# smoggy-P/gym-Drone2D-ActivePerception

Measured on AMD Instinct MI355X. Metric: env-steps/sec (batched) at 10 agents, map_id=1, higher is better.
Workload: dtype f64

## Files before the change

gym-drone2d-activeperception_amd/csrc/d2d_hip.hip:

```cpp
#include <hip/hip_runtime.h>
#include <math.h>
#include <stdint.h>
#include <stdio.h>
#include <stdlib.h>
#include <string.h>
#include <type_traits>

#if defined(__HIP_DEVICE_COMPILE__)
#define D2D_AS __attribute__((address_space(1)))
#endif
#include "../../include/d2d.h"
#include "../../include/d2d_hooks.h"
#include "../../include/d2d_stepped.h"
#include "../../include/d2d_swept.h"

#define D2D_TAN_QUAL __device__ __forceinline__
#define D2D_TAN_TBL_QUAL __device__ const
#include "d2d_tan.h"
#define D2D_LOG_QUAL __device__ __forceinline__
#define D2D_LOG_TBL_QUAL __device__ const
#define D2D_RNG_QUAL __device__ __forceinline__
#include "d2d_rng.h"

#define WAVE 64
// ... 1885 lines not shown
  }
}

__global__ __launch_bounds__(WAVE *WAVES_PER_BLOCK) void k_reset(d2d_cfg c, d2d_state s, d2d_state init,
                                                                 const unsigned char *mask, int mask_stride) {
  const int lane = threadIdx.x & (WAVE - 1), wv = threadIdx.x / WAVE;
  const int e = blockIdx.x * WAVES_PER_BLOCK + wv;
  if (e >= c.B) return;
  if (mask && !mask[(size_t)e * mask_stride]) return;
  reset_env(c, s, init, (size_t)e, lane);
}

__global__ void k_tan(const double *in, double *out, long long n) {
  const long long i = (long long)blockIdx.x * blockDim.x + threadIdx.x;
  if (i < n) out[i] = d2d_tan(in[i]);
}

__global__ void k_log(const double *x, double *out, long long n) {
  const long long i = (long long)blockIdx.x * blockDim.x + threadIdx.x;
  if (i < n) out[i] = d2d_log(x[i]);
}

__global__ __launch_bounds__(WAVE) void k_rng_draw(uint32_t *rng, const int *m, double *out, int max_m) {
  const int lane = threadIdx.x;
  uint32_t *st = rng + (size_t)blockIdx.x * D2D_RNG_WORDS;
  double *o = out + (size_t)blockIdx.x * max_m * 2;
  const int mb = __builtin_amdgcn_readfirstlane(min(max(m[blockIdx.x], 0), max_m));
  int pos = __builtin_amdgcn_readfirstlane((int)st[D2D_RNG_POS]);
  const bool bad = !rng_pos_ok(pos);
  int got = 0, regen = 0;
  if (!bad)
    got = rng_wave_pairs(st, pos, regen, d2d_rng_regen_cap(mb), mb, lane, [&](int q, double v0, double v1) {
      o[(size_t)q * 2] = v0;
      o[(size_t)q * 2 + 1] = v1;
    });
  for (int k = got + lane; k < max_m; k += WAVE) o[(size_t)k * 2] = o[(size_t)k * 2 + 1] = k < mb ? __builtin_nan("") : 0.0;
  if (!bad) rng_wave_store(st, pos, got, regen, lane);
}

#include "d2d_plugins.h"

__global__ void k_atan2(const double *y, const double *x, double *out, long long n) {
  const long long i = (long long)blockIdx.x * blockDim.x + threadIdx.x;
  if (i < n) out[i] = d2d_atan2(y[i], x[i]);
}

struct ClosedArgs {
  d2d_cfg c;
  d2d_state s;
  d2d_plan p;
  d2d_state init;
  int on_done, nsteps;
  int obs_every;
};
static_assert(sizeof(ClosedArgs) <= D2D_LAUNCH_ARGS_BYTES, "d2d_plan.launch_args (D2D_LAUNCH_ARGS_BYTES) is too small for the parked launch arguments");

__global__ void k_closed_args(ClosedArgs *dst, d2d_cfg c, d2d_state s, d2d_plan p, d2d_state init, int on_done, int nsteps, int obs_every) {
  if (threadIdx.x == 0 && blockIdx.x == 0) {
    dst->c = c;
    dst->s = s;
    dst->p = p;
    dst->init = init;
    dst->on_done = on_done;
    dst->nsteps = nsteps;
    dst->obs_every = obs_every;
  }
}

template <int SPEC>
__host__ __device__ inline int closed_wave_bytes(const d2d_cfg &c, const d2d_plan &p, int wpb) {
  int b = make_geom(c, wpb, spec_ncap(SPEC), spec_full(SPEC)).wave_bytes;
  const int pb = plan_wave_bytes(c.N, p.nu, p.n_sample, c.W, c.H), gb = p.gaze == D2D_GAZE_OXFORD ? gaze_geom(c, p).wave_bytes : 0;
  b = b > pb ? b : pb;
  b = b > gb ? b : gb;
  return (b + 15) & ~15;
}


#if defined(__HIP_DEVICE_COMPILE__)
typedef const ClosedArgs __attribute__((address_space(4))) *ArgsPtr;
#else
typedef const ClosedArgs *ArgsPtr;
#endif

struct PhaseIn {
  ArgsPtr a;
  int e, off, lane;
};
__device__ __forceinline__ PhaseIn phase_enter(const ClosedArgs *ap, int e_, int lds_off_) {
  const unsigned long long v = (unsigned long long)ap;
  unsigned int lo = __builtin_amdgcn_readfirstlane((unsigned int)v), hi = __builtin_amdgcn_readfirstlane((unsigned int)(v >> 32));
  int e = __builtin_amdgcn_readfirstlane(e_), off = __builtin_amdgcn_readfirstlane(lds_off_);
  int lane = threadIdx.x & (WAVE - 1);
  asm volatile("; phase" : "+s"(lo), "+s"(hi), "+s"(e), "+s"(off), "+v"(lane));
  PhaseIn in;
  in.a = (ArgsPtr)(((unsigned long long)hi << 32) | lo);
  in.e = e;
  in.off = off;
  in.lane = lane;
  return in;
}
template <bool PDEF, typename F>
__device__ __forceinline__ auto with_plan(ArgsPtr a, F f) {
  if constexpr (PDEF) {
    d2d_plan p = a->p;
    plan_default_apply(p);
    return f(p);
  } else {
    return f(a->p);
  }
}


template <int SPEC, bool PDEF>
__device__ __forceinline__ int ph_plan_quick(const ClosedArgs *ap, int e_, int lds_off_) {
  const PhaseIn in_ = phase_enter(ap, e_, lds_off_);
  const ArgsPtr a = in_.a;
  const int e = in_.e, lane = in_.lane;
  char *base = d2d_lds + in_.off;
  d2d_cfg c = a->c;
  if (!spec_generic(SPEC)) spec_default_apply(c);
  if constexpr (SPEC == 1 || SPEC == 2) {
    constexpr int cap = spec_ncap(SPEC);
    __builtin_assume(c.N <= cap);
  }
  const bool need = with_plan<PDEF>(a, [&](const d2d_plan &p) __attribute__((always_inline)) { return plan_env_quick(c, a->s, p, e, lane, base); });
  wave_sync_global();
  return need ? 1 : 0;
}

template <int SPEC, bool PDEF>
__device__ __forceinline__ void ph_plan_search(const ClosedArgs *ap, int e_, int lds_off_) {
  const PhaseIn in_ = phase_enter(ap, e_, lds_off_);
  const ArgsPtr a = in_.a;
  const int e = in_.e, lane = in_.lane;
  char *base = d2d_lds + in_.off;
  d2d_cfg c = a->c;
  if (!spec_generic(SPEC)) spec_default_apply(c);
  if constexpr (SPEC == 1 || SPEC == 2) {
    constexpr int cap = spec_ncap(SPEC);
    __builtin_assume(c.N <= cap);
  }
  with_plan<PDEF>(a, [&](const d2d_plan &p) __attribute__((always_inline)) { plan_env_search<PDEF>(c, a->s, p, e, lane, base); });
  wave_sync_global();
}

__host__ __device__ constexpr uint32_t hidden_stages(uint32_t stages) { return stages & ~(uint32_t)D2D_ST_OBS; }
__host__ __device__ constexpr bool late_obs_of(uint32_t stages) { return (stages & D2D_ST_COLLIDE) && !(stages & D2D_ST_OBS); }


template <int SPEC, bool PDEF, uint32_t ACT = D2D_ST_ACT>
__device__ __forceinline__ int ph_plan_act(const ClosedArgs *ap, int e_, int lds_off_, int &walls_ok) {
  const PhaseIn in_ = phase_enter(ap, e_, lds_off_);
  const ArgsPtr a = in_.a;
  const int e = in_.e, lane = in_.lane;
  char *base = d2d_lds + in_.off;
  d2d_cfg c = a->c;
  if (!spec_generic(SPEC)) spec_default_apply(c);
  if constexpr (SPEC == 1 || SPEC == 2) {
    constexpr int cap = spec_ncap(SPEC);
    __builtin_assume(c.N <= cap);
  }
  double4 w_head;
  int wk = __builtin_amdgcn_readfirstlane(walls_ok);
  asm volatile("; phase" : "+s"(wk));
  const bool need = with_plan<PDEF>(a, [&](const d2d_plan &p) __attribute__((always_inline)) { return plan_env_quick(c, a->s, p, e, lane, base, &w_head, &wk); });
  walls_ok = __builtin_amdgcn_readfirstlane(wk);
  if (need) {
    wave_sync_global();
    return -1;
  }
  wave_sync_lds();
  StepIn in;
  in.action = 0.0;
  in.ok = true;
  in.has_wp = true;
  in.wp[0] = w_head.x; in.wp[1] = w_head.y; in.wp[2] = w_head.z; in.wp[3] = w_head.w; in.wp[4] = 0.0; in.wp[5] = 0.0;
  const int wpb = (int)(blockDim.x / WAVE);
  const Geom g = make_geom(c, wpb, spec_ncap(SPEC), spec_full(SPEC));
  const LdsView L = carve(base, g, c.L);
  EnvRegs r;
  run_env<spec_full(SPEC), spec_wide(SPEC), spec_cone(SPEC), spec_tiled(SPEC)>(c, a->s, e, lane, ACT, g, L, a->s.action[e], r, 0, true, &in, late_obs_of(ACT));
  if (lane == 0) store_regs(a->s, e, r);
  wave_sync_global();
  return r.done;
}

template <int SPEC, bool PDEF, uint32_t STAGES>
__device__ __forceinline__ int ph_gaze_stages(const ClosedArgs *ap, int e_, int lds_off_, int t_, int done_, int &dyn_gate, bool dyn_vis_) {
  const PhaseIn in_ = phase_enter(ap, e_, lds_off_);
  const ArgsPtr a = in_.a;
  const int e = in_.e, lane = in_.lane;
  int tstep = __builtin_amdgcn_readfirstlane(t_), known_done = __builtin_amdgcn_readfirstlane(done_);
  asm volatile("; phase" : "+s"(tstep), "+s"(known_done));
  int dgate = 2;
  const int dvis = dyn_vis_ ? 1 : 0;
  if constexpr (spec_full(SPEC)) {
    dgate = __builtin_amdgcn_readfirstlane(dyn_gate);
    asm volatile("; phase" : "+s"(dgate));
  }
  char *base = d2d_lds + in_.off;
  d2d_cfg c = a->c;
  if (!spec_generic(SPEC)) spec_default_apply(c);
#ifdef D2D_CHAIN_PROF
  const unsigned long long pp0 = __builtin_amdgcn_s_memtime();
#endif
  with_plan<PDEF>(a, [&](const d2d_plan &p) __attribute__((always_inline)) {
    gaze_env<true, PDEF>(c, a->s, p, a->init, a->on_done == D2D_DONE_RESET, e, lane, base, known_done);
  });
  wave_sync_global();
#ifdef D2D_CHAIN_PROF
  D2D_PHASE_ADD(0, pp0);
  const unsigned long long pp1 = __builtin_amdgcn_s_memtime();
#endif
  const int wpb = (int)(blockDim.x / WAVE);
  const Geom g = make_geom(c, wpb, spec_ncap(SPEC), spec_full(SPEC));
  const LdsView L = carve(base, g, c.L);
  EnvRegs r;
  load_regs(a->s, e, r);
  const size_t noise_off = c.noise_rows > 1 ? (size_t)((c.noise_row0 + tstep) % c.noise_rows) * c.B * c.N * 2 : 0;
  if constexpr (spec_full(SPEC)) {
    run_env<true, spec_wide(SPEC), spec_cone(SPEC), spec_tiled(SPEC)>(c, a->s, e, lane, STAGES, g, L, a->s.action[e], r, noise_off, false, nullptr, late_obs_of(STAGES), &dgate, dvis != 0, dgate == 1 && dvis == 0);
    dyn_gate = __builtin_amdgcn_readfirstlane(dgate);
  } else {
    run_env<spec_full(SPEC), spec_wide(SPEC), spec_cone(SPEC), spec_tiled(SPEC)>(c, a->s, e, lane, STAGES, g, L, a->s.action[e], r, noise_off, false, nullptr, late_obs_of(STAGES));
  }
  if (lane == 0) store_regs(a->s, e, r);
  wave_sync_global();
#ifdef D2D_CHAIN_PROF
  D2D_PHASE_ADD(1, pp1);
#endif
  return r.done;
}

template <int SPEC, uint32_t STAGES>
__device__ __forceinline__ int ph_stages(const ClosedArgs *ap, int e_, int lds_off_) {
  const PhaseIn in_ = phase_enter(ap, e_, lds_off_);
  const ArgsPtr a = in_.a;
  const int e = in_.e, lane = in_.lane;
  char *base = d2d_lds + in_.off;
  d2d_cfg c = a->c;
  if (!spec_generic(SPEC)) spec_default_apply(c);
  const int wpb = (int)(blockDim.x / WAVE);
  const Geom g = make_geom(c, wpb, spec_ncap(SPEC), spec_full(SPEC));
  const LdsView L = carve(base, g, c.L);
  EnvRegs r;
  run_env<spec_full(SPEC), spec_wide(SPEC), spec_cone(SPEC), spec_tiled(SPEC)>(c, a->s, e, lane, STAGES, g, L, a->s.action[e], r, 0, true, nullptr, late_obs_of(STAGES));
  if (lane == 0) store_regs(a->s, e, r);
  wave_sync_global();
  return r.done;
}

template <int SPEC, bool PDEF = false>
__global__ __launch_bounds__(WAVE *WAVES_PER_BLOCK, D2D_MIN_WAVES) void k_closed(const ClosedArgs *__restrict__ a) {
  static_assert(!PDEF || SPEC == 1, "the plan's defaults are folded into the few-agent kernel of the default geometry only");
  const int wv = __builtin_amdgcn_readfirstlane(threadIdx.x / WAVE);
  const int wpb = (int)(blockDim.x / WAVE);
  const int e = blockIdx.x * wpb + wv;
  if (e >= a->c.B) return;
  d2d_cfg c = a->c;
  if (!spec_generic(SPEC)) spec_default_apply(c);
  int off;
  bool split;
  if constexpr (PDEF) {
    d2d_plan p = a->p;
    plan_default_apply(p);
    off = wv * closed_wave_bytes<SPEC>(c, p, wpb);
    split = p.planner == D2D_PLAN_PRIMITIVE;
  } else {
    off = wv * closed_wave_bytes<SPEC>(c, a->p, wpb);
    split = a->p.planner == D2D_PLAN_PRIMITIVE;
  }
  const int nsteps = a->nsteps;
  const bool freeze = a->on_done == D2D_DONE_FREEZE;
  const bool obs_every = a->obs_every != 0;
  const bool dyn_defer = spec_full(SPEC) && !obs_every && !freeze, auto_reset = a->on_done == D2D_DONE_RESET;
  int dyn_gate = dyn_defer ? 0 : 2;
  int nsearch = 0;
  int walls_ok = 0;
#ifdef D2D_CHAIN_PROF
  const unsigned long long cp0 = __builtin_amdgcn_s_memtime();
  unsigned long long cps = 0;
#endif
  int flag_done = a->s.flags[(size_t)e * 4 + D2D_F_DONE] != 0 ? 1 : 0;
#pragma unroll 1
  for (int t = 0; t < nsteps; ++t) {
    if (freeze && flag_done != 0) break;
    const bool visible = obs_every || t == nsteps - 1;
    if (dyn_defer && auto_reset && flag_done != 0) dyn_gate = 0;
    if (split) {
      if (nsearch * 32 > t + 16) __builtin_amdgcn_s_setprio(2); else __builtin_amdgcn_s_setprio(0);
      ph_gaze_stages<SPEC, PDEF, D2D_ST_PERCEIVE>(a, e, off, t, flag_done, dyn_gate, visible);
#ifdef D2D_CHAIN_PROF
      const unsigned long long q0 = __builtin_amdgcn_s_memtime();
#endif
      const int pa = __builtin_amdgcn_readfirstlane(visible ? ph_plan_act<SPEC, PDEF, D2D_ST_ACT>(a, e, off, walls_ok)
                                                            : ph_plan_act<SPEC, PDEF, hidden_stages(D2D_ST_ACT)>(a, e, off, walls_ok));
#ifdef D2D_CHAIN_PROF
      D2D_PHASE_ADD(2, q0);
#endif
      if (pa < 0) {
#ifdef D2D_CHAIN_PROF
        const unsigned long long s0 = __builtin_amdgcn_s_memtime();
#endif
        ph_plan_search<SPEC, PDEF>(a, e, off);
        nsearch += 1;
        walls_ok = 0;
#ifdef D2D_CHAIN_PROF
        cps += __builtin_amdgcn_s_memtime() - s0;
        D2D_PHASE_ADD(3, s0);
        const unsigned long long a0 = __builtin_amdgcn_s_memtime();
#endif
        flag_done = __builtin_amdgcn_readfirstlane(visible ? ph_stages<SPEC, D2D_ST_ACT>(a, e, off)
                                                           : ph_stages<SPEC, hidden_stages(D2D_ST_ACT)>(a, e, off));
#ifdef D2D_CHAIN_PROF
        D2D_PHASE_ADD(4, a0);
#endif
      } else {
        flag_done = pa;
      }
    } else {
      flag_done = __builtin_amdgcn_readfirstlane(visible ? ph_gaze_stages<SPEC, PDEF, D2D_ST_ALL>(a, e, off, t, flag_done, dyn_gate, true)
                                                         : ph_gaze_stages<SPEC, PDEF, hidden_stages(D2D_ST_ALL)>(a, e, off, t, flag_done, dyn_gate, false));
    }
  }
#ifdef D2D_CHAIN_PROF
  if ((threadIdx.x & (WAVE - 1)) == 0 && a->p.plan_stat) {
    const unsigned long long tot = __builtin_amdgcn_s_memtime() - cp0;
    a->p.plan_stat[(size_t)e * 4 + 1] = (int)(tot >> 4);
    a->p.plan_stat[(size_t)e * 4 + 2] = (int)(cps >> 4);
  }
#endif
}

#include "d2d_swept.h"

thread_local char g_err[256] = "";

int fail(int code, const char *msg) {
  snprintf(g_err, sizeof g_err, "%s", msg);
  return code;
}

constexpr size_t LDS_SOFT = 64 * 1024, LDS_HARD = 160 * 1024;

template <typename K>
void lds_optin(K kernel, size_t bytes) {
  if (bytes > LDS_SOFT) (void)hipFuncSetAttribute((const void *)kernel, hipFuncAttributeMaxDynamicSharedMemorySize, (int)bytes);
}

int launched() {
  const hipError_t err = hipGetLastError();
  return err == hipSuccess ? 0 : fail(-3, hipGetErrorString(err));
}

dim3 env_grid(int B, int wpb = WAVES_PER_BLOCK) { return dim3((B + wpb - 1) / wpb); }
dim3 env_block(int wpb = WAVES_PER_BLOCK) { return dim3(WAVE * wpb); }

// ... 286 lines not shown

int d2d_reset(const d2d_cfg *c, const d2d_state *s, const d2d_state *init, const uint8_t *mask, void *stream) {
  return reset_launch(c, s, init, mask, 1, stream);
}

int d2d_gaze_stage(const d2d_cfg *c, const d2d_state *s, const d2d_plan *p, void *stream) {
  int rc = plan_check(c, s, p);
  if (rc) return rc;
  return gaze_launch(c, s, p, nullptr, false, stream);
}

int d2d_plan_stage(const d2d_cfg *c, const d2d_state *s, const d2d_plan *p, void *stream) {
  int rc = plan_check(c, s, p);
  if (rc) return rc;
  return plan_launch(c, s, p, false, stream);
}

int d2d_gaze_stage_live(const d2d_cfg *c, const d2d_state *s, const d2d_plan *p, void *stream) {
  int rc = plan_check(c, s, p);
  if (rc) return rc;
  return gaze_launch(c, s, p, nullptr, true, stream);
}

int d2d_plan_stage_live(const d2d_cfg *c, const d2d_state *s, const d2d_plan *p, void *stream) {
  int rc = plan_check(c, s, p);
  if (rc) return rc;
  return plan_launch(c, s, p, true, stream);
}

#define D2D_SWEPT_ENTRY_POINTS
#include "d2d_swept.h"

int d2d_plan_reset(const d2d_cfg *c, const d2d_plan *p, const uint8_t *mask, int32_t mask_stride, void *stream) {
  if (!c || !p) return fail(-1, "null cfg/plan");
  if (c->abi_version != D2D_ABI_VERSION) return fail(-2, "ABI version mismatch");
  return plan_reset_launch(c, p, mask, mask_stride, stream);
}

int d2d_closed_loop(const d2d_cfg *c, const d2d_state *s, const d2d_plan *p, int32_t nsteps, int32_t on_done,
                    const d2d_state *init, void *stream) {
  int rc = plan_check(c, s, p);
  if (rc) return rc;
  if (nsteps < 0) return fail(-1, "closed_loop: bad step count");
  if (on_done < D2D_DONE_CONTINUE || on_done > D2D_DONE_FREEZE) return fail(-1, "closed_loop: bad on_done");
  const bool auto_reset = on_done == D2D_DONE_RESET;
  if (auto_reset && !snapshot_complete(init)) return fail(-1, "closed_loop: D2D_DONE_RESET needs the snapshot");
  if (c->B == 0 || nsteps == 0) return 0;
  if (c->planner_mode == D2D_PLANNER_EXTERNAL && p->launch_args && (p->planner == D2D_PLAN_PRIMITIVE || p->gaze != D2D_GAZE_NONE)) {
    const Launch l = pick_launch(*c, p);
    if (l.wpb >= 1) {
      ClosedArgs *dev = (ClosedArgs *)p->launch_args;
      const char *obs_env = getenv("D2D_OBS_EVERY_STEP");
      const bool obs_every = obs_env && obs_env[0] == '1' && obs_env[1] == '\0';
      hipLaunchKernelGGL(k_closed_args, dim3(1), dim3(64), 0, (hipStream_t)stream, dev, *c, *s, *p, auto_reset ? *init : *s,
                         (int)on_done, (int)nsteps, obs_every ? 1 : 0);
      auto launch = [&](auto kernel) {
        lds_optin(kernel, l.lds());
        hipLaunchKernelGGL(kernel, env_grid(c->B, l.wpb), env_block(l.wpb), l.lds(), (hipStream_t)stream, (const ClosedArgs *)dev);
      };
      const char *fold_env = getenv("D2D_PLAN_FOLD");
      const bool fold_off = fold_env && fold_env[0] == '0' && fold_env[1] == '\0';
      if (l.spec == 1 && !fold_off && plan_default_matches(*c, *p)) launch(k_closed<1, true>);
      else with_spec(l.spec, [&](auto S) { launch(k_closed<decltype(S)::value>); });
      return launched();
    }
  }
  const bool split = p->planner == D2D_PLAN_PRIMITIVE;
  const uint32_t skip = on_done == D2D_DONE_FREEZE ? D2D_ST_SKIP_DONE : 0;
  for (int32_t t = 0; t < nsteps; ++t) {
    if ((rc = gaze_launch(c, s, p, auto_reset ? init : nullptr, skip != 0, stream))) return rc;
    d2d_state sn = *s;
    sn.noise = noise_row(c, s, t);
    if (split) {
      if ((rc = launch_stages(c, &sn, D2D_ST_PERCEIVE | skip, stream))) return rc;
      if ((rc = plan_launch(c, s, p, skip != 0, stream))) return rc;
      if ((rc = launch_stages(c, s, D2D_ST_ACT | skip, stream))) return rc;
    } else if ((rc = launch_stages(c, &sn, D2D_ST_ALL | skip, stream))) {
      return rc;
    }
  }
  return 0;
}

int d2d_launch_shape(const d2d_cfg *c, const d2d_plan *p, int32_t out[4]) {
  if (!c || !out) return fail(-1, "launch_shape: null argument");
  if (c->abi_version != D2D_ABI_VERSION) return fail(-2, "ABI version mismatch");
  Launch l = pick_launch(*c, p);
  if (p && (!p->launch_args || c->planner_mode != D2D_PLANNER_EXTERNAL)) l.wpb = 0;
  out[0] = l.wpb;
  out[1] = (int32_t)l.lds();
  out[2] = out[1] > 0 ? (int32_t)(LDS_HARD / (size_t)out[1]) : 0;
  out[3] = spec_full(l.spec) ? 1 : 0;
  return 0;
}

int d2d_sincos_array(const double *in, double *so, double *co, int64_t n, void *stream) {
  return launch_array(k_sincos, n, n > 0 && (!in || !so || !co), "sincos_array: bad arguments", stream, in, so, co);
}

int d2d_tan_array(const double *in, double *out, int64_t n, void *stream) {
  return launch_array(k_tan, n, n > 0 && (!in || !out), "tan_array: bad arguments", stream, in, out);
}

int d2d_atan2_array(const double *y, const double *x, double *out, int64_t n, void *stream) {
  return launch_array(k_atan2, n, n > 0 && (!y || !x || !out), "atan2_array: bad arguments", stream, y, x, out);
}

int d2d_log_array(const double *x, double *out, int64_t n, void *stream) {
// ... 16 lines not shown
```

gym-drone2d-activeperception_amd/csrc/d2d_plugins.h:

```cpp

#define D2D_SINCOS_QUAL __device__ __forceinline__
#define D2D_SINCOS_TBL_QUAL __device__ const
#include "d2d_sincos.h"
#define D2D_ATAN2_QUAL __device__ __forceinline__
#define D2D_ATAN2_TBL_QUAL __device__ const
#include "d2d_atan2.h"
#define D2D_POW2_QUAL __device__ __forceinline__
#define D2D_POW2_TBL_QUAL __device__ const
#include "d2d_pow2.h"

__device__ __forceinline__ double norm2(double x, double y) { return sqrt(__builtin_fma(y, y, x * x)); }

__device__ __forceinline__ double shfl_f64(double v, int src) {
  int lo = __double2loint(v), hi = __double2hiint(v);
  lo = __shfl(lo, src, WAVE);
  hi = __shfl(hi, src, WAVE);
  return __hiloint2double(hi, lo);
}

template <int N>
__device__ __forceinline__ double row_shl_f64(double v) {
  int lo = __double2loint(v), hi = __double2hiint(v);
  lo = __builtin_amdgcn_update_dpp(lo, lo, 0x100 + N, 0xf, 0xf, false);
  hi = __builtin_amdgcn_update_dpp(hi, hi, 0x100 + N, 0xf, 0xf, false);
// ... 157 lines not shown
#endif
__device__ __forceinline__ double *traj_boxes(const d2d_plan &p, int e) {
  return p.traj_box ? (double *)p.traj_box + (size_t)e * ((p.traj_cap + WAVE - 1) / WAVE) * 4 : nullptr;
}

#define LH_N 1024
#define LH_MAX 896

#ifdef D2D_SEARCH_PROF
__device__ unsigned long long d2d_search_prof[16];
#define SP_T(var)                                              \
  do {                                                         \
    asm volatile("s_waitcnt vmcnt(0) lgkmcnt(0)" ::: "memory"); \
    var = __builtin_amdgcn_s_memtime();                        \
  } while (0)
#define SP_ADD(idx, t0, t1) \
  do {                      \
    spacc[idx] += (t1) - (t0); \
  } while (0)
#define SP_FLUSH()                                                            \
  do {                                                                        \
    if (e == 0 && lane == 0)                                                  \
      for (int spi = 0; spi < 16; ++spi) d2d_search_prof[spi] += spacc[spi]; \
  } while (0)
#else
#define SP_T(var) do { } while (0)
#define SP_ADD(idx, t0, t1) do { } while (0)
#define SP_FLUSH() do { } while (0)
#endif

template <int N>
struct IntC {
  static constexpr int value = N;
};

struct SearchLds {
  int *chain;
  double *us;
  double *st;
  double *pc;
  double *rv;
  long long *rk;
  int *ri;
  int *misc;
  double *tot;
  int ntot;
  unsigned long long *prow;
  unsigned short *lh;
};

__host__ __device__ inline int search_lds_nodes(int N) { return N > 64 ? 256 : 512; }
__host__ __device__ inline bool search_wall_rows(int W, int H) { return W <= 64 && H <= 64; }

template <bool PDEF = false>
__device__ int plan_search(const d2d_cfg &c, const d2d_state &s, const d2d_plan &p, int e, int lane, const TrkView &T,
                           const SearchLds &S, const unsigned char *__restrict__ dm, double inv_scale) {
  const double H = p.horizon;
  const NodeRecs nd = {p.nodes + (size_t)e * p.node_cap * D2D_NODE_F};
  int *__restrict__ tab = p.hash + (size_t)e * p.hash_cap;
  double *__restrict__ traj = p.traj + (size_t)e * p.traj_cap * 4;
  int *stat = p.plan_stat + (size_t)e * 4;
  int *chain = S.chain;
  const unsigned int hmask = (unsigned int)p.hash_cap - 1u;
  const double tx = s.target[(size_t)e * 2], ty = s.target[(size_t)e * 2 + 1];
  const double *dr = s.drone + (size_t)e * D2D_DF;

  unsigned long long spa = 0, spb = 0;
  (void)spa; (void)spb;
#ifdef D2D_SEARCH_PROF
  unsigned long long spacc[16] = {0, 0, 0, 0, 0, 0, 0, 0, 0, 0, 0, 0, 0, 0, 0, 0};
#endif
  SP_T(spa);
  for (int i = lane; i < p.nu; i += WAVE) S.us[i] = p.u_space[i];
  {
    const FastDiv fdu(p.nu);
    for (int i = lane; i < p.nu * p.nu; i += WAVE) {
      int ia, ja;
      fdu.divmod(i, ia, ja);
      const double ax = p.u_space[ia], ay = p.u_space[ja];
      S.pc[i] = (ax * ax + ay * ay) / 100;
    }
  }
  for (int i = lane; i < 2 * p.n_sample; i += WAVE) S.st[i] = p.sample_t[i];
  {
    uint4 *lh128 = (uint4 *)S.lh;
    for (int i = lane; i < LH_N / 8; i += WAVE) lh128[i] = make_uint4(0u, 0u, 0u, 0u);
  }
  const bool int_walls = c.scale == 10.0 && c.W_px <= 81919.0 && c.H_px <= 81919.0 && c.W_px == floor(c.W_px) &&
                         c.H_px == floor(c.H_px) && c.W_px >= 1.0 && c.H_px >= 1.0 && p.safe_dist >= 0.0 &&
                         p.safe_dist <= 1048576.0 && p.safe_dist == floor(p.safe_dist);
  const int safe_i = int_walls ? (int)p.safe_dist : 0, wpx_i = int_walls ? (int)c.W_px : 1, hpx_i = int_walls ? (int)c.H_px : 1;
  const int kcell = safe_i / 10;
  const bool rows = S.prow != nullptr && int_walls && c.W <= 64 && c.H <= 64 && c.W_px == 10.0 * (double)c.W &&
                    c.H_px == 10.0 * (double)c.H && safe_i == 10 * kcell && 2 * kcell <= min(c.W, c.H);
  if (rows) {
    int olo = 0, ohi = 0;
    unsigned long long *orow = (unsigned long long *)S.rk;
    const int nb = c.W * c.H;
    if (c.grid_tile == 0 && (nb & 3) == 0 && (((size_t)dm) & 3) == 0) {
      orow[lane] = 0ull;
      const unsigned int *src = (const unsigned int *)dm;
      const FastDiv fdh(c.H);
      for (int d0 = 0; d0 < nb / 4; d0 += 10 * WAVE) {
        unsigned int x[10];
#pragma unroll
        for (int u = 0; u < 10; ++u) {
          const int idx = d0 + u * WAVE + lane;
          x[u] = src[min(idx, nb / 4 - 1)];
        }
// ... 452 lines not shown
            }
            if (atomicCAS(&lh32[h >> 1], w, w | (ent << sh)) == w) break;
          }
        } else {
          unsigned int hh = h;
          for (int guard = 0; guard < p.hash_cap; ++guard) {
            if (atomicCAS(&tab[hh], 0, myslot + 1) == 0) break;
            hh = (hh + 1) & hmask;
          }
        }
      }
      nn += nnew;
      open_n += nnew;
      SP_T(sp7);
      SP_ADD(6, sp6, sp7);
      if (p0 + WAVE < nprim) wave_sync_global();
      else wave_sync_lds();
      SP_T(sp8);
      SP_ADD(7, sp7, sp8);
      SP_ADD(8, sp0, sp8);
#ifdef D2D_SEARCH_PROF
      spacc[9] += 1;
#endif
    }
    if (overflow) break;
  }
  if (lane == 0) {
    stat[0] += 1;
    stat[1] = expansions;
    stat[2] = nn;
    if (overflow) stat[3] = 1;
  }
  if (goal < 0 || overflow) {
    SP_FLUSH();
    return -1;
  }
  SP_T(spa);
  int depth = 0;
  for (int q = goal; q != 0 && depth <= 128; q = meta_parent(nd.rec(q)[NR_META])) depth += 1;
  if (depth * p.n_ts > p.traj_cap || depth > 128) {
    if (lane == 0) stat[3] = 1;
    return -1;
  }
  if (lane == 0) {
    int q = goal;
    for (int lvl = depth - 1; lvl >= 0; --lvl) {
      chain[lvl] = q;
      q = meta_parent(nd.rec(q)[NR_META]);
    }
  }
  wave_sync_lds();
  const int total = depth * p.n_ts;
  double *tbox = traj_boxes(p, e);
  for (int w0 = 0; w0 < total; w0 += WAVE) {
    const int w = w0 + lane;
    double ox = 0.0, oy = 0.0;
    if (w < total) {
      const int lvl = w / p.n_ts, mi = w - lvl * p.n_ts;
      const int q = chain[lvl];
      const double *rq = nd.rec(q);
      const int par = meta_parent(rq[NR_META]);
      const double2 acc = ld2(rq + NR_ACC);
      const double hx = acc.x / 2, hy = acc.y / 2;
      const double t = p.traj_t[3 * mi], t2 = p.traj_t[3 * mi + 1], tt = p.traj_t[3 * mi + 2];
      const double2 pp = ld2(nd.rec(par) + NR_POS), pv = ld2(nd.rec(par) + NR_VEL);
      double *o = traj + (size_t)w * 4;
      ox = rint(__builtin_fma(t2, hx, pp.x + t * pv.x));
      oy = rint(__builtin_fma(t2, hy, pp.y + t * pv.y));
      o[0] = ox;
      o[1] = oy;
      o[2] = pv.x + tt * hx;
      o[3] = pv.y + tt * hy;
    }
    if (tbox) {
      const bool on = w < total;
      const double xlo = wave_fmin(on ? ox : 1e300), ylo = wave_fmin(on ? oy : 1e300);
      const double xhi = wave_fmax(on ? ox : -1e300), yhi = wave_fmax(on ? oy : -1e300);
      if (lane == 0) {
        st2(tbox + 4 * (w0 / WAVE), xlo, ylo);
        st2(tbox + 4 * (w0 / WAVE) + 2, xhi, yhi);
      }
    }
  }
  SP_T(spb);
  SP_ADD(11, spa, spb);
#ifdef D2D_SEARCH_PROF
  spacc[12] += 1;
#endif
  SP_FLUSH();
  return total;
}

__host__ __device__ inline int plan_wave_bytes(int N, int nu, int n_sample, int W, int H) {
  const int ncap = ((N > 0 ? N : 1) + 3) & ~3;
  const int nu4 = ((nu + 3) & ~3) + ((nu * nu + 3) & ~3), ns4 = (2 * n_sample + 3) & ~3;
  const int rowb = search_wall_rows(W, H) ? 8 * 64 : 0;
  return 5 * 8 * ncap + 8 * (nu4 + ns4) + 8 * 64 + 8 * 64 + 4 * 64 + 128 * 4 + 16 + 8 * search_lds_nodes(N) + rowb + 2 * LH_N;
}

__device__ __forceinline__ void plan_carve(const d2d_cfg &c, const d2d_plan &p, char *base, TrkView &T, SearchLds &S) {
  const int N = c.N, ncap = ((N > 0 ? N : 1) + 3) & ~3;
  T.mx = (double *)base;
  T.my = T.mx + ncap;
  T.vx = T.my + ncap;
  T.vy = T.vx + ncap;
  T.lim = T.vy + ncap;
  S.us = T.lim + ncap;
  S.pc = S.us + ((p.nu + 3) & ~3);
  S.st = S.pc + ((p.nu * p.nu + 3) & ~3);
  S.rv = S.st + ((2 * p.n_sample + 3) & ~3);
  S.rk = (long long *)(S.rv + 64);
  S.ri = (int *)(S.rk + 64);
  S.chain = S.ri + 64;
  S.misc = S.chain + 128;
  S.tot = (double *)(S.misc + 4);
  S.ntot = search_lds_nodes(N);
  unsigned long long *after = (unsigned long long *)(S.tot + S.ntot);
  S.prow = search_wall_rows(c.W, c.H) ? after : nullptr;
  S.lh = (unsigned short *)(after + (search_wall_rows(c.W, c.H) ? 64 : 0));
}

__device__ __forceinline__ void plan_emit(const d2d_state &s, const d2d_plan &p, int e, int lane, int head, int stored, int ok,
                                          const double4 *w_head = nullptr) {
  if (lane == 0) {
    const double *traj = p.traj + (size_t)e * p.traj_cap * 4;
// ... 123 lines not shown
          double mx[4], my[4], vx[4], vy[4], lim[4];
#pragma unroll
          for (int u = 0; u < 4; ++u) {
            mx[u] = T.mx[q + u]; my[u] = T.my[q + u]; vx[u] = T.vx[q + u]; vy[u] = T.vy[q + u]; lim[u] = T.lim[q + u];
          }
#pragma unroll
          for (int u = 0; u < 4; ++u) {
            const double ex = mx[u] + ti * vx[u], ey = my[u] + ti * vy[u];
            const double dx = ex - wx, dy = ey - wy;
            bad = bad | ((q + u < nact) & (__builtin_fma(dy, dy, dx * dx) <= lim[u]));
          }
        }
      }
    };
    if (__builtin_expect(chunked, 0)) {
      for (unsigned long long m = cmask; m; m &= m - 1ull) {
        const int cc = c_lo + __ffsll((long long)m) - 1;
        visit((cc << 6) + lane, cc == c_lo);
      }
    } else {
      for (int a0 = head; a0 < stored; a0 += WAVE) visit(a0 + lane, a0 == head);
    }
    if (__builtin_expect(chunked && n > 0, 0)) {
      const int hl = head & 63;
      w_first = make_double4(readlane_f64(w_first.x, hl), readlane_f64(w_first.y, hl), readlane_f64(w_first.z, hl), readlane_f64(w_first.w, hl));
    }
    const bool replan = __any(bad);
    if (replan) head = stored = 0;
    if (walls_ok) *walls_ok = (!replan && n > 0 && n < 2560 && (walls_full || walls_known)) ? 1 : 0;
  }
  if (stored - head == 0) {
    int q0 = 0;
    for (int k0 = 0; k0 < N; k0 += WAVE) {
      const int k = k0 + lane;
      const bool act = k < N && s.active[(size_t)e * N + k] != 0;
      const unsigned long long am = __ballot(act);
      if (act) T.lim[q0 + __popcll(am & ((1ull << lane) - 1ull))] = sq_threshold(c.drone_radius + p.trk_radius[(size_t)e * N + k] + 5 + c.sigma);
      q0 += __popcll(am);
    }
    if (lane == 0) {
      hdr[0] = 0;
      hdr[1] = 0;
      S.misc[0] = nact;
    }
    wave_sync_lds();
    return true;
  }
  plan_emit(s, p, e, lane, head, stored, 1, &w_first);
  if (w_head_out)
    *w_head_out = make_double4(readlane_f64(w_first.x, 0), readlane_f64(w_first.y, 0), readlane_f64(w_first.z, 0), readlane_f64(w_first.w, 0));
  return false;
}

template <bool PDEF = false>
__device__ __forceinline__ void plan_env_search(const d2d_cfg &c, const d2d_state &s, const d2d_plan &p, int e, int lane, char *base) {
  TrkView T;
  SearchLds S;
  plan_carve(c, p, base, T, S);
  T.n = S.misc[0];
  const double inv_scale = 1.0 / c.scale;
  const unsigned char *__restrict__ dm = s.dmap + (size_t)e * grid_bytes(c);
  __builtin_amdgcn_s_setprio(3);
  const int found = plan_search<PDEF>(c, s, p, e, lane, T, S, dm, inv_scale);
  __builtin_amdgcn_s_setprio(0);
  wave_sync_global();
  plan_emit(s, p, e, lane, 0, found > 0 ? found : 0, found >= 0 ? 1 : 0);
}

__device__ __forceinline__ void plan_env(const d2d_cfg &c, const d2d_state &s, const d2d_plan &p, int e, int lane, char *base) {
  if (plan_env_quick(c, s, p, e, lane, base)) plan_env_search(c, s, p, e, lane, base);
}

__global__ __launch_bounds__(WAVE *WAVES_PER_BLOCK) void k_plan(d2d_cfg c, d2d_state s, d2d_plan p, int skip_done) {
  const int lane = threadIdx.x & (WAVE - 1);
  const int wv = __builtin_amdgcn_readfirstlane(threadIdx.x / WAVE);
  const int e = blockIdx.x * (int)(blockDim.x / WAVE) + wv;
  if (e >= c.B) return;
  if (skip_done && s.flags[(size_t)e * 4 + D2D_F_DONE] != 0) return;
  plan_env(c, s, p, e, lane, d2d_lds + (size_t)wv * plan_wave_bytes(c.N, p.nu, p.n_sample, c.W, c.H));
}

__device__ __forceinline__ long long dkey(double x) {
  const long long b = __double_as_longlong(x);
  return b ^ ((b >> 63) & 0x7FFFFFFFFFFFFFFFll);
}

__device__ __forceinline__ bool acos_le(const d2d_plan &p, double q) {
  if (!(fabs(q) <= 1.0)) return false;
  const long long k = dkey(q);
  if (k >= p.acos_key_lo + 64) return true;
  if (k < p.acos_key_lo) return false;
  return ((p.acos_mask >> (int)(k - p.acos_key_lo)) & 1ull) != 0ull;
}

struct ViewCone {
  double cy, sy;
};

__device__ __forceinline__ bool view_cell(const d2d_plan &p, double depth2, double quick, double x0, double y0,
                                          const ViewCone &v, double x, double y) {
  const double a = x0 - x, b = y0 - y;
  const double d2 = a * a + b * b;
  if (d2 <= 0.0) return true;
  if (!(d2 <= depth2)) return false;
  const double dot = (x - x0) * v.cy + (y - y0) * v.sy;
  if (quick > 0.0) {
    const double lhs = dot * dot, rhs = quick * d2;
    if (dot > 0.0 && lhs > rhs * (1.0 + 1e-12) && lhs < d2 * (1.0 - 1e-12)) return true;
    if (dot <= 0.0 || lhs < rhs * (1.0 - 1e-12)) return false;
  }
  return acos_le(p, dot / sqrt(d2));
}

__device__ __forceinline__ void plan_reset_env(const d2d_cfg &c, const d2d_plan &p, size_t e, int lane) {
  const size_t N = (size_t)(c.N > 0 ? c.N : 1), WH = (size_t)c.W * c.H;
  if (p.traj_hdr && lane < 2) p.traj_hdr[e * 2 + lane] = 0;
  for (size_t k = lane; k < N; k += WAVE) {
    if (p.trk_radius && p.trk_radius0) p.trk_radius[e * N + k] = p.trk_radius0[e * N + k];
    if (p.trk_prev) p.trk_prev[e * N + k] = 0;
// ... 180 lines not shown
  const double t1 = (speed2 * owl_unseen(h - d_v, half, hp, hn)) * flight_unknown;

  int nact = 0;
  for (int b0 = 0; b0 < N; b0 += WAVE) {
    const int t = b0 + lane;
    nact += __popcll(__ballot(t < N && s.active[(size_t)e * N + t] != 0));
  }
  const double *kf = s.kf + (size_t)e * N * D2D_KF;
  double t2 = 0.0;
  for (int j0 = 0; j0 < nact; j0 += WAVE) {
    const int j = j0 + lane;
    int mine = 0, seen = 0;
    for (int b0 = 0; b0 < N; b0 += WAVE) {
      const int t = b0 + lane;
      unsigned long long m = __ballot(t < N && s.active[(size_t)e * N + t] != 0);
      while (m) {
        if (seen == j) mine = b0 + __ffsll((long long)m) - 1;
        ++seen;
        m &= m - 1;
      }
    }
    double d_o = 0.0, pull = 0.0;
    if (j < nact) {
      const double *ma = kf + (size_t)mine * D2D_KF, *mj = kf + (size_t)j * D2D_KF;
      d_o = d2d_atan2(ma[1] - y0, ma[0] - x0) * rad2deg;
      pull = norm2(mj[2], mj[3]) / norm2(mj[0] - x0, mj[1] - y0);
    }
    const int cnt = min(nact - j0, WAVE);
    for (int q = 0; q < cnt; ++q) t2 += shfl_f64(pull, q) * owl_unseen(h - shfl_f64(d_o, q), half, hp, hn);
  }

  double cost = __builtin_fma(t0, 0.2, 0.0);
  cost = __builtin_fma(t1, 0.9, cost);
  cost = __builtin_fma(t2, 1.0, cost);
  cost = __builtin_fma(u_l, 0.1, cost);
  cost = __builtin_fma(tab[D2D_OWL_T_TURN + min(lane, D2D_OWL_NRATE - 1)], 0.0, cost);

  int best = 0;
  double best_c = shfl_f64(cost, 0);
  for (int a = 1; a < D2D_OWL_NRATE; ++a) {
    const double v = shfl_f64(cost, a);
    if (best_c == best_c && (v < best_c || v != v)) {
      best = a;
      best_c = v;
    }
  }
  if (lane == 0) {
    st[D2D_OWL_S_RATE] = tab[D2D_OWL_T_RATE + best];
    st[D2D_OWL_S_LEFT] = tab[D2D_OWL_T_HOLD];
    act[e] = tab[D2D_OWL_T_ACT + best];
  }
}

template <bool OWL, bool PDEF = false>
__device__ __forceinline__ void gaze_env(const d2d_cfg &c, const d2d_state &s, const d2d_plan &p, const d2d_state &init,
                                         int auto_reset, int e, int lane, char *base, int known_done = -1, bool reset_rng = true) {
  constexpr int NA = PDEF ? 6 : 7;
  const bool oxford = p.gaze == D2D_GAZE_OXFORD;
  const GazeGeom g = gaze_geom(c, p);
  const double *dr = s.drone + (size_t)e * D2D_DF;
  const int *hdr = p.traj_hdr + (size_t)e * 2;
  const int was_done = !auto_reset ? 0 : (known_done >= 0 ? known_done : (int)s.flags[(size_t)e * 4 + D2D_F_DONE]);
  double x0 = dr[D2D_D_X], y0 = dr[D2D_D_Y], yaw = dr[D2D_D_YAW];
  int steps = s.counters[(size_t)e * D2D_CF + D2D_C_STEPS];
  int head = 0, stored = 0;
  double ys_l = 0.0, tob_l = 0.0;
  if (oxford) {
    head = hdr[0];
    stored = hdr[1];
    ys_l = p.yaw_space[min(lane & 7, max(p.n_yaw, 1) - 1)];
    tob_l = p.tobs_tab[min(lane, p.tobs_len - 1)];
  }
  if (was_done != 0) {
    reset_env(c, s, init, (size_t)e, lane, reset_rng);
    plan_reset_env(c, p, (size_t)e, lane);
    wave_sync_global();
    x0 = dr[D2D_D_X]; y0 = dr[D2D_D_Y]; yaw = dr[D2D_D_YAW];
    steps = s.counters[(size_t)e * D2D_CF + D2D_C_STEPS];
    if (oxford) {
      head = hdr[0];
      stored = hdr[1];
    }
  }
  if (!oxford) {
    if (p.gaze == D2D_GAZE_LOOKAHEAD || p.gaze == D2D_GAZE_LOOKGOAL) heading_gaze_env(c, s, p, e, lane, x0, y0, yaw);
    if constexpr (OWL) {
      if (p.gaze == D2D_GAZE_OWL) owl_gaze_env(c, s, p, e, lane, x0, y0, yaw);
    }
    return;
  }
#ifdef D2D_CHAIN_PROF
  unsigned long long gz_t = __builtin_amdgcn_s_memtime();
#endif
  double *rew = (double *)base;
  const int nnode = g.nnode;
  double *lsum = rew + g.ncell;
  const int lsum_doubles = max(p.n_yaw * nnode, (g.ncell + 1) / 2);
  double *stk = lsum + lsum_doubles;
  double *tobl = stk + 16;
  int *swi = (int *)(tobl + D2D_TOBS_LDS);
  int *swl = (int *)lsum;
  int *pwl = swi + g.ncell;
  int *pwp = pwl + 4 * g.nleaf;
  unsigned char *cm = (unsigned char *)(pwp + g.ntree);
  int *rng = (int *)(cm + ((g.ncell + 7) & ~7));
  const int W = c.W, H = c.H;
  const double deg2rad = 0x1.1df46a2529d39p-6;
  const double depth2 = c.depth * c.depth;
  const double inv_scale = 1.0 / c.scale;
// ... 25 lines not shown
      v = lane < 8 ? r : -r;
    }
    vdir[2 * a + (lane >> 3)] = v;
  }
  double span_deg;
  {
    double m = lane < p.n_yaw ? fabs(ys_l) * c.dt : 0.0;
    m = fmax(m, row_shl_f64<1>(m));
    m = fmax(m, row_shl_f64<2>(m));
    m = fmax(m, row_shl_f64<4>(m));
    span_deg = readlane_f64(m, 0);
  }
  wave_sync_lds();
  ViewCone cone7;
  cone7.cy = vdir[14];
  cone7.sy = vdir[15];
  GZ(0);
  const float w_own = (float)p.half_fov + 2.0f * 0.0174533f, w_all = (float)p.half_fov + ((float)span_deg + 3.0f) * 0.0174533f;
  const bool boxes = w_all < 1.518f && span_deg <= 90.0;
  {
    const int bi = (int)floor((x0 - c.depth) * inv_scale) - 1, bj = (int)floor((y0 - c.depth) * inv_scale) - 1;
    CellBox b;
    b.i_lo = bi; b.i_hi = bi + g.bbn - 1; b.j_lo = bj; b.j_hi = bj + g.bbn - 1;
    if (boxes) {
      const CellBox sb = sector_box(x0, y0, c.depth, inv_scale, cone7.cy, cone7.sy, __cosf(w_own), __sinf(w_own));
      b.i_lo = max(b.i_lo, sb.i_lo); b.i_hi = min(b.i_hi, sb.i_hi); b.j_lo = max(b.j_lo, sb.j_lo); b.j_hi = min(b.j_hi, sb.j_hi);
    }
    b.i_lo = max(b.i_lo, 0); b.i_hi = min(b.i_hi, W - 1); b.j_lo = max(b.j_lo, 0); b.j_hi = min(b.j_hi, H - 1);
    const int nc = b.j_hi - b.j_lo + 1, nsub = (b.i_hi - b.i_lo + 1) * nc;
    if (nc > 0 && nsub > 0) {
      const FastDiv fds(nc);
      for (int q0 = 0; q0 < nsub; q0 += WAVE) {
        const int q = q0 + lane;
        int r, cc;
        fds.divmod(q, r, cc);
        const int i = b.i_lo + r, j = b.j_lo + cc;
        if (q < nsub) {
          if (view_cell(p, depth2, quick, x0, y0, cone7, (double)i * c.scale, (double)j * c.scale)) seen[i * H + j] = call;
        }
      }
    }
  }
#if defined(D2D_GAZE_ABL) && D2D_GAZE_ABL == 1
  if (lane == 0) act[e] = 0.0;
  return;
#endif
  GZ(1);
  if (n == 0) {
    if (lane == 0) act[e] = 0.0;
    return;
  }
  const double hx = hxy.x, hy = hxy.y;
  const int bi = (int)floor((hx - c.depth) * inv_scale) - 1, bj = (int)floor((hy - c.depth) * inv_scale) - 1;
  for (int q = lane; q < g.ncell; q += WAVE) swi[q] = -1;
  wave_sync_lds();
  {
    const int c_lo = head >> 6, c_hi = (stored - 1) >> 6;
    const double *tbox = traj_boxes(p, e);
    unsigned long long cmask = 0ull;
    const bool chunked = tbox != nullptr && c_hi - c_lo < 64 && c_hi - c_lo >= D2D_TRAJ_PRUNE_CHUNKS;
    if (__builtin_expect(chunked, 0)) {
      bool need = false;
      if (c_lo + lane <= c_hi) {
        const double2 lo = ld2(tbox + 4 * (c_lo + lane)), hi = ld2(tbox + 4 * (c_lo + lane) + 2);
        const double bx0 = (double)bi * c.scale, bx1 = (double)(bi + g.bbn) * c.scale;
        const double by0 = (double)bj * c.scale, by1 = (double)(bj + g.bbn) * c.scale;
        need = (hi.x >= bx0) & (lo.x < bx1) & (hi.y >= by0) & (lo.y < by1);
      }
      cmask = __ballot(need);
    }
    auto visit = [&](int a) {
      if (a >= head && a < stored) {
        const int i = a - head;
        const double2 wxy = ld2(traj + (size_t)a * 4);
        const int ci = cell_fast(wxy.x, c.scale, inv_scale), cj = cell_fast(wxy.y, c.scale, inv_scale);
        const int r = ci - bi, cc = cj - bj;
        if (ci >= 0 && ci < W && cj >= 0 && cj < H && r >= 0 && r < g.bbn && cc >= 0 && cc < g.bbn) atomicMax(&swi[r * g.bbn + cc], i);
      }
    };
    if (__builtin_expect(chunked, 0)) {
      for (unsigned long long m = cmask; m; m &= m - 1ull) visit(((c_lo + __ffsll((long long)m) - 1) << 6) + lane);
    } else {
      for (int a0 = head; a0 < stored; a0 += WAVE) visit(a0 + lane);
    }
  }
  wave_sync_global();
  GZ(2);
#if defined(D2D_GAZE_ABL) && D2D_GAZE_ABL == 2
  if (lane == 0) act[e] = 0.0;
  return;
#endif
  double wide2 = 0.0;
  if (boxes) {
    const double cwd = (double)__cosf(w_all) * 0.98;
    wide2 = cwd * cwd;
  }
  for (int k = lane; k < (g.ncell + 3) / 4; k += WAVE) ((unsigned int *)cm)[k] = 0u;
  int nlive = 0;
  {
    CellBox b;
    b.i_lo = bi; b.i_hi = bi + g.bbn - 1; b.j_lo = bj; b.j_hi = bj + g.bbn - 1;
    if (boxes) {
      const CellBox sb = sector_box(hx, hy, c.depth, inv_scale, cone7.cy, cone7.sy, __cosf(w_all), __sinf(w_all));
      b.i_lo = max(b.i_lo, sb.i_lo); b.i_hi = min(b.i_hi, sb.i_hi); b.j_lo = max(b.j_lo, sb.j_lo); b.j_hi = min(b.j_hi, sb.j_hi);
    }
    b.i_lo = max(b.i_lo, 0); b.i_hi = min(b.i_hi, W - 1); b.j_lo = max(b.j_lo, 0); b.j_hi = min(b.j_hi, H - 1);
    const int nc = b.j_hi - b.j_lo + 1, nsub = (nc > 0 && b.i_hi >= b.i_lo) ? (b.i_hi - b.i_lo + 1) * nc : 0;
    const FastDiv fds(nc > 0 ? nc : 1);
    for (int q0 = 0; q0 < nsub; q0 += WAVE) {
      const int qs = q0 + lane;
      int r, cc;
      fds.divmod(qs, r, cc);
      const int i = b.i_lo + r, j = b.j_lo + cc;
      const int q = (i - bi) * g.bbn + (j - bj);
      bool live = false;
      if (qs < nsub) {
        const double ca = hx - (double)i * c.scale, cb = hy - (double)j * c.scale;
        const double d2 = ca * ca + cb * cb;
        const double dm = (-ca) * cone7.cy + (-cb) * cone7.sy;
        const bool sector = (wide2 <= 0.0) | (d2 <= 0.0) | ((dm > 0.0) & (dm * dm >= wide2 * d2));
        live = (d2 <= depth2) & sector;
      }
      const unsigned long long lm = __ballot(live);
      if (live) swl[nlive + __popcll(lm & ((1ull << lane) - 1ull))] = q;
      nlive += __popcll(lm);
    }
  }
  if (lane == 0) {
    rng[0] = 0;
    rng[1] = 0;
    rng[2] = 0;
    rng[3] = 0;
  }
  wave_sync_lds();
#if defined(D2D_GAZE_ABL) && D2D_GAZE_ABL == 3
  if (lane == 0) act[e] = 0.0;
  return;
#endif
  GZ(3);
#ifndef D2D_GAZE_EXACT_ONLY
  double qa[NA];
#pragma unroll
  for (int a = 0; a < NA; ++a) qa[a] = 0.0;
#endif
  bool any_hot = false;
  for (int l0 = 0; l0 < nlive; l0 += 4 * WAVE) {
    int qq[4], sn[4];
#pragma unroll
    for (int u = 0; u < 4; ++u) {
      qq[u] = swl[min(l0 + u * WAVE + lane, nlive - 1)];
      int r, cc;
      fdb.divmod(qq[u], r, cc);
      sn[u] = seen[(bi + r) * H + (bj + cc)];
    }
    double tobs[4];
#pragma unroll
    for (int u = 0; u < 4; ++u) {
      const int k = call - min(sn[u], call);
      tobs[u] = sn[u] > 0 ? tobl[min(k, D2D_TOBS_LDS - 1)] : 5.0;
    }
    if (__any(tobl[D2D_TOBS_LDS - 1] < 1.0)) {
#pragma unroll
      for (int u = 0; u < 4; ++u) tobs[u] = sn[u] > 0 ? p.tobs_tab[call - min(sn[u], call)] : p.tobs_tab[p.tobs_len + call];
    }
#pragma unroll
    for (int u = 0; u < 4; ++u) {
      if (l0 + u * WAVE + lane < nlive) {
        const int q = qq[u];
        int r, cc;
        fdb.divmod(q, r, cc);
        const int i = bi + r, j = bj + cc;
        const int si = swi[q];
        const double sw = si >= 0 ? (double)si * c.dt : 0.0;
        const bool stale = tobs[u] >= 0.5;
        double rw = (1.0 * tobs[u] < 1.0) ? 1.0 * tobs[u] : 1.0;
        rw = ((sw > 3.0) & stale) ? 1000.0 : rw;
        rw = ((sw > 0.0) & (sw <= 3.0) & stale) ? 1000000.0 : rw;
        const double x = (double)i * c.scale, y = (double)j * c.scale;
        const double ca = hx - x, cb = hy - y;
        const double d2 = ca * ca + cb * cb;
        unsigned int bits = 0, rare = 0;
        if (d2 <= 0.0) {
          bits = (1u << p.n_yaw) - 1u;
        } else {
          const double dxv = x - hx, dyv = y - hy;
          const double rhs = quick * d2, hi = rhs * (1.0 + 1e-12), lo = rhs * (1.0 - 1e-12), top = d2 * (1.0 - 1e-12);
#pragma unroll
          for (int a = 0; a < NA; ++a) {
            if (a < p.n_yaw) {
              const double dot = dxv * vdir[2 * a] + dyv * vdir[2 * a + 1];
              const double sq = dot * fabs(dot);
              const bool inside = (quick > 0.0) & (sq > hi) & (sq < top);
              const bool outside = (quick > 0.0) & (sq < lo);
              bits |= inside ? (1u << a) : 0u;
              rare |= (inside | outside) ? 0u : (1u << a);
            }
          }
          if (rare) {
            const double rs = sqrt(d2);
            for (unsigned int m = rare; m; m &= m - 1) {
              const int a = __ffs((int)m) - 1;
              const double dot = dxv * vdir[2 * a] + dyv * vdir[2 * a + 1];
              bits |= acos_le(p, dot / rs) ? (1u << a) : 0u;
            }
          }
        }
        const bool hot = (bits != 0u) & (rw != 0.0);
        rew[q] = rw;
        cm[q] = hot ? (unsigned char)bits : (unsigned char)0;
#ifndef D2D_GAZE_EXACT_ONLY
        {
          const int hbits = hot ? (int)bits : 0;
#pragma unroll
          for (int a = 0; a < NA; ++a) {
            const double view = __hiloint2double(((hbits << (31 - a)) >> 31) & 0x3ff00000, 0);
            qa[a] = __builtin_fma(rw, view, qa[a]);
          }
        }
#endif
        any_hot = any_hot | hot;
      }
    }
  }
  wave_sync_lds();
#if defined(D2D_GAZE_ABL) && D2D_GAZE_ABL == 4
// ... 340 lines not shown
```

Measured before the change: 104.0 million.

## Build per-cell trajectory index once per search and reuse in gaze

After: 105.1 million (median of 6 runs). +1.0%, better.

```diff
diff --git a/gym-drone2d-activeperception_amd/csrc/d2d_hip.hip b/gym-drone2d-activeperception_amd/csrc/d2d_hip.hip
--- a/gym-drone2d-activeperception_amd/csrc/d2d_hip.hip
+++ b/gym-drone2d-activeperception_amd/csrc/d2d_hip.hip
@@ -1961,10 +1961,11 @@
   d2d_state init;
   int on_done, nsteps;
   int obs_every;
+  int traj_once;
 };
 static_assert(sizeof(ClosedArgs) <= D2D_LAUNCH_ARGS_BYTES, "d2d_plan.launch_args (D2D_LAUNCH_ARGS_BYTES) is too small for the parked launch arguments");
 
-__global__ void k_closed_args(ClosedArgs *dst, d2d_cfg c, d2d_state s, d2d_plan p, d2d_state init, int on_done, int nsteps, int obs_every) {
+__global__ void k_closed_args(ClosedArgs *dst, d2d_cfg c, d2d_state s, d2d_plan p, d2d_state init, int on_done, int nsteps, int obs_every, int traj_once) {
   if (threadIdx.x == 0 && blockIdx.x == 0) {
     dst->c = c;
     dst->s = s;
@@ -1973,6 +1974,7 @@
     dst->on_done = on_done;
     dst->nsteps = nsteps;
     dst->obs_every = obs_every;
+    dst->traj_once = traj_once;
   }
 }
 
@@ -2039,7 +2041,7 @@
 }
 
 template <int SPEC, bool PDEF>
-__device__ __forceinline__ void ph_plan_search(const ClosedArgs *ap, int e_, int lds_off_) {
+__device__ __forceinline__ int ph_plan_search(const ClosedArgs *ap, int e_, int lds_off_) {
   const PhaseIn in_ = phase_enter(ap, e_, lds_off_);
   const ArgsPtr a = in_.a;
   const int e = in_.e, lane = in_.lane;
@@ -2050,8 +2052,11 @@
     constexpr int cap = spec_ncap(SPEC);
     __builtin_assume(c.N <= cap);
   }
-  with_plan<PDEF>(a, [&](const d2d_plan &p) __attribute__((always_inline)) { plan_env_search<PDEF>(c, a->s, p, e, lane, base); });
+  const int found = with_plan<PDEF>(a, [&](const d2d_plan &p) __attribute__((always_inline)) {
+    return plan_env_search<PDEF, spec_full(SPEC)>(c, a->s, p, e, lane, base, a->traj_once != 0);
+  });
   wave_sync_global();
+  return found;
 }
 
 __host__ __device__ constexpr uint32_t hidden_stages(uint32_t stages) { return stages & ~(uint32_t)D2D_ST_OBS; }
@@ -2096,12 +2101,18 @@
 }
 
 template <int SPEC, bool PDEF, uint32_t STAGES>
-__device__ __forceinline__ int ph_gaze_stages(const ClosedArgs *ap, int e_, int lds_off_, int t_, int done_, int &dyn_gate, bool dyn_vis_) {
+__device__ __forceinline__ int ph_gaze_stages(const ClosedArgs *ap, int e_, int lds_off_, int t_, int done_, int &dyn_gate, bool dyn_vis_,
+                                              int plane_ = 0) {
   const PhaseIn in_ = phase_enter(ap, e_, lds_off_);
   const ArgsPtr a = in_.a;
   const int e = in_.e, lane = in_.lane;
   int tstep = __builtin_amdgcn_readfirstlane(t_), known_done = __builtin_amdgcn_readfirstlane(done_);
   asm volatile("; phase" : "+s"(tstep), "+s"(known_done));
+  int plane = 0;
+  if constexpr (spec_full(SPEC)) {
+    plane = __builtin_amdgcn_readfirstlane(plane_);
+    asm volatile("; phase" : "+s"(plane));
+  }
   int dgate = 2;
   const int dvis = dyn_vis_ ? 1 : 0;
   if constexpr (spec_full(SPEC)) {
@@ -2115,7 +2126,7 @@
   const unsigned long long pp0 = __builtin_amdgcn_s_memtime();
 #endif
   with_plan<PDEF>(a, [&](const d2d_plan &p) __attribute__((always_inline)) {
-    gaze_env<true, PDEF>(c, a->s, p, a->init, a->on_done == D2D_DONE_RESET, e, lane, base, known_done);
+    gaze_env<true, PDEF, spec_full(SPEC)>(c, a->s, p, a->init, a->on_done == D2D_DONE_RESET, e, lane, base, known_done, true, plane);
   });
   wave_sync_global();
 #ifdef D2D_CHAIN_PROF
@@ -2187,6 +2198,7 @@
   int dyn_gate = dyn_defer ? 0 : 2;
   int nsearch = 0;
   int walls_ok = 0;
+  int plane_ok = 0;
 #ifdef D2D_CHAIN_PROF
   const unsigned long long cp0 = __builtin_amdgcn_s_memtime();
   unsigned long long cps = 0;
@@ -2199,7 +2211,7 @@
     if (dyn_defer && auto_reset && flag_done != 0) dyn_gate = 0;
     if (split) {
       if (nsearch * 32 > t + 16) __builtin_amdgcn_s_setprio(2); else __builtin_amdgcn_s_setprio(0);
-      ph_gaze_stages<SPEC, PDEF, D2D_ST_PERCEIVE>(a, e, off, t, flag_done, dyn_gate, visible);
+      ph_gaze_stages<SPEC, PDEF, D2D_ST_PERCEIVE>(a, e, off, t, flag_done, dyn_gate, visible, plane_ok);
 #ifdef D2D_CHAIN_PROF
       const unsigned long long q0 = __builtin_amdgcn_s_memtime();
 #endif
@@ -2212,7 +2224,8 @@
 #ifdef D2D_CHAIN_PROF
         const unsigned long long s0 = __builtin_amdgcn_s_memtime();
 #endif
-        ph_plan_search<SPEC, PDEF>(a, e, off);
+        const int found = __builtin_amdgcn_readfirstlane(ph_plan_search<SPEC, PDEF>(a, e, off));
+        plane_ok = (spec_full(SPEC) && found > 0 && a->traj_once != 0) ? 1 : 0;
         nsearch += 1;
         walls_ok = 0;
 #ifdef D2D_CHAIN_PROF
@@ -2605,8 +2618,12 @@
       ClosedArgs *dev = (ClosedArgs *)p->launch_args;
       const char *obs_env = getenv("D2D_OBS_EVERY_STEP");
       const bool obs_every = obs_env && obs_env[0] == '1' && obs_env[1] == '\0';
+      const char *once_env = getenv("D2D_TRAJ_ONCE");
+      const bool once_off = once_env && once_env[0] == '0' && once_env[1] == '\0';
+      const bool traj_once = !once_off && spec_full(l.spec) && p->planner == D2D_PLAN_PRIMITIVE && p->gaze == D2D_GAZE_OXFORD && p->hash &&
+                             (long long)p->hash_cap >= (long long)c->W * c->H;
       hipLaunchKernelGGL(k_closed_args, dim3(1), dim3(64), 0, (hipStream_t)stream, dev, *c, *s, *p, auto_reset ? *init : *s,
-                         (int)on_done, (int)nsteps, obs_every ? 1 : 0);
+                         (int)on_done, (int)nsteps, obs_every ? 1 : 0, traj_once ? 1 : 0);
       auto launch = [&](auto kernel) {
         lds_optin(kernel, l.lds());
         hipLaunchKernelGGL(kernel, env_grid(c->B, l.wpb), env_block(l.wpb), l.lds(), (hipStream_t)stream, (const ClosedArgs *)dev);
diff --git a/gym-drone2d-activeperception_amd/csrc/d2d_plugins.h b/gym-drone2d-activeperception_amd/csrc/d2d_plugins.h
--- a/gym-drone2d-activeperception_amd/csrc/d2d_plugins.h
+++ b/gym-drone2d-activeperception_amd/csrc/d2d_plugins.h
@@ -233,9 +233,9 @@
 __host__ __device__ inline int search_lds_nodes(int N) { return N > 64 ? 256 : 512; }
 __host__ __device__ inline bool search_wall_rows(int W, int H) { return W <= 64 && H <= 64; }
 
-template <bool PDEF = false>
+template <bool PDEF = false, bool PLANE = false>
 __device__ int plan_search(const d2d_cfg &c, const d2d_state &s, const d2d_plan &p, int e, int lane, const TrkView &T,
-                           const SearchLds &S, const unsigned char *__restrict__ dm, double inv_scale) {
+                           const SearchLds &S, const unsigned char *__restrict__ dm, double inv_scale, bool plane = false) {
   const double H = p.horizon;
   const NodeRecs nd = {p.nodes + (size_t)e * p.node_cap * D2D_NODE_F};
   int *__restrict__ tab = p.hash + (size_t)e * p.hash_cap;
@@ -794,6 +794,13 @@
   wave_sync_lds();
   const int total = depth * p.n_ts;
   double *tbox = traj_boxes(p, e);
+  const int ncells = c.W * c.H;
+  if constexpr (PLANE) {
+    if (plane) {
+      for (int i = lane; i < ncells && i < p.hash_cap; i += WAVE) tab[i] = -1;
+      wave_sync_global();
+    }
+  }
   for (int w0 = 0; w0 < total; w0 += WAVE) {
     const int w = w0 + lane;
     double ox = 0.0, oy = 0.0;
@@ -813,6 +820,13 @@
       o[1] = oy;
       o[2] = pv.x + tt * hx;
       o[3] = pv.y + tt * hy;
+      if constexpr (PLANE) {
+        if (plane) {
+          const int ci = cell_fast(ox, c.scale, inv_scale), cj = cell_fast(oy, c.scale, inv_scale);
+          const int ix = ci * c.H + cj;
+          if (ci >= 0 && ci < c.W && cj >= 0 && cj < c.H && ix < ncells && ix < p.hash_cap) atomicMax(&tab[ix], w);
+        }
+      }
     }
     if (tbox) {
       const bool on = w < total;
@@ -1042,8 +1056,9 @@
   return false;
 }
 
-template <bool PDEF = false>
-__device__ __forceinline__ void plan_env_search(const d2d_cfg &c, const d2d_state &s, const d2d_plan &p, int e, int lane, char *base) {
+template <bool PDEF = false, bool PLANE = false>
+__device__ __forceinline__ int plan_env_search(const d2d_cfg &c, const d2d_state &s, const d2d_plan &p, int e, int lane, char *base,
+                                               bool plane = false) {
   TrkView T;
   SearchLds S;
   plan_carve(c, p, base, T, S);
@@ -1051,10 +1066,11 @@
   const double inv_scale = 1.0 / c.scale;
   const unsigned char *__restrict__ dm = s.dmap + (size_t)e * grid_bytes(c);
   __builtin_amdgcn_s_setprio(3);
-  const int found = plan_search<PDEF>(c, s, p, e, lane, T, S, dm, inv_scale);
+  const int found = plan_search<PDEF, PLANE>(c, s, p, e, lane, T, S, dm, inv_scale, plane);
   __builtin_amdgcn_s_setprio(0);
   wave_sync_global();
   plan_emit(s, p, e, lane, 0, found > 0 ? found : 0, found >= 0 ? 1 : 0);
+  return found;
 }
 
 __device__ __forceinline__ void plan_env(const d2d_cfg &c, const d2d_state &s, const d2d_plan &p, int e, int lane, char *base) {
@@ -1341,9 +1357,10 @@
   }
 }
 
-template <bool OWL, bool PDEF = false>
+template <bool OWL, bool PDEF = false, bool PLANE = false>
 __device__ __forceinline__ void gaze_env(const d2d_cfg &c, const d2d_state &s, const d2d_plan &p, const d2d_state &init,
-                                         int auto_reset, int e, int lane, char *base, int known_done = -1, bool reset_rng = true) {
+                                         int auto_reset, int e, int lane, char *base, int known_done = -1, bool reset_rng = true,
+                                         int plane_ok = 0) {
   constexpr int NA = PDEF ? 6 : 7;
   const bool oxford = p.gaze == D2D_GAZE_OXFORD;
   const GazeGeom g = gaze_geom(c, p);
@@ -1475,9 +1492,11 @@
   }
   const double hx = hxy.x, hy = hxy.y;
   const int bi = (int)floor((hx - c.depth) * inv_scale) - 1, bj = (int)floor((hy - c.depth) * inv_scale) - 1;
-  for (int q = lane; q < g.ncell; q += WAVE) swi[q] = -1;
-  wave_sync_lds();
-  {
+  const bool from_plane = PLANE && plane_ok != 0;
+  const int *__restrict__ swp = p.hash + (size_t)e * p.hash_cap;
+  if (!from_plane) {
+    for (int q = lane; q < g.ncell; q += WAVE) swi[q] = -1;
+    wave_sync_lds();
     const int c_lo = head >> 6, c_hi = (stored - 1) >> 6;
     const double *tbox = traj_boxes(p, e);
     unsigned long long cmask = 0ull;
@@ -1568,13 +1587,17 @@
 #endif
   bool any_hot = false;
   for (int l0 = 0; l0 < nlive; l0 += 4 * WAVE) {
-    int qq[4], sn[4];
+    int qq[4], sn[4], sp[4];
 #pragma unroll
     for (int u = 0; u < 4; ++u) {
       qq[u] = swl[min(l0 + u * WAVE + lane, nlive - 1)];
       int r, cc;
       fdb.divmod(qq[u], r, cc);
       sn[u] = seen[(bi + r) * H + (bj + cc)];
+      if constexpr (PLANE) {
+        sp[u] = -1;
+        if (from_plane) sp[u] = swp[min(max((bi + r) * H + (bj + cc), 0), W * H - 1)];
+      }
     }
     double tobs[4];
 #pragma unroll
@@ -1593,7 +1616,9 @@
         int r, cc;
         fdb.divmod(q, r, cc);
         const int i = bi + r, j = bj + cc;
-        const int si = swi[q];
+        int si;
+        if constexpr (PLANE) si = from_plane ? (sp[u] >= head ? sp[u] - head : -1) : swi[q];
+        else si = swi[q];
         const double sw = si >= 0 ? (double)si * c.dt : 0.0;
         const bool stale = tobs[u] >= 0.5;
         double rw = (1.0 * tobs[u] < 1.0) ? 1.0 * tobs[u] : 1.0;
```
